# D-Hank/NeRF-tiny

Hardware: AMD Instinct MI355X
Metric: rays/sec (64 coarse + 128 fine samples), lego 400x400 (higher is better)
Workload: dtype f32

## Files before the change

### nerf-tiny_amd/csrc/field_fwd_reg.hip

```cpp
#include "field_common.h"
#include <type_traits>

namespace nerf {

constexpr int RM = 32;

template <int I0, int I1, class F>
__device__ __forceinline__ void static_for(F&& f) {
  if constexpr (I0 < I1) {
    f(std::integral_constant<int, I0>{});
    static_for<I0 + 1, I1>(f);
  }
}

template <int NFT>
struct WStage {
  float4 w[NFT];
};

template <int KB, int NFT>
__device__ __forceinline__ void stage_load(const float4* __restrict__ seg_lane, int kb, WStage<NFT>& s) {
#pragma unroll
  for (int f = 0; f < NFT; ++f) s.w[f] = seg_lane[(size_t)(f * KB + kb) * 64];
}

__device__ __forceinline__ float relu1(float x) { return __int_as_float(max(__float_as_int(x), 0)); }

__device__ __forceinline__ float f4c(const float4& v, int c) { return c == 0 ? v.x : (c == 1 ? v.y : (c == 2 ? v.z : v.w)); }

typedef int lds_i32 __attribute__((address_space(3), may_alias));
typedef int i32x4v __attribute__((ext_vector_type(4), may_alias));
typedef __attribute__((address_space(3))) i32x4v lds_i32x4;
constexpr int RELU_LDS_DWORDS = 2 * 4 * 64 * 4;
constexpr int COL_LDS_DWORDS = 3 * HALF + 4;
struct ReluLds {
  lds_i32* w;
  lds_i32* m[4];
};
__device__ __forceinline__ ReluLds relu_lds(lds_i32* base, int lane) {
  ReluLds L;
  L.w = base + 4 * lane;
#pragma unroll
  for (int c = 0; c < 4; ++c) L.m[c] = base + 4 * lane + ((c + (lane >> 3)) & 3);
  return L;
}
__device__ __forceinline__ float4 lds_ld4(const lds_i32* p) {
  const i32x4v v = *reinterpret_cast<const lds_i32x4*>(p);
  return make_float4(__int_as_float(v[0]), __int_as_float(v[1]), __int_as_float(v[2]), __int_as_float(v[3]));
}
template <typename DST>
__device__ __forceinline__ void relu_lds_op(const ReluLds& L, const f32x16& src, DST& dst, int dst0, int slot, int i) {
  const int g = i / 6, j = i - 6 * g, off = (slot * 4 + g) * 256;
  if (j == 0) {
    const i32x4v v = {__float_as_int(src[4 * g]), __float_as_int(src[4 * g + 1]), __float_as_int(src[4 * g + 2]), __float_as_int(src[4 * g + 3])};
    *reinterpret_cast<lds_i32x4*>(L.w + off) = v;
  } else if (j < 5) {
    __hip_atomic_fetch_max(L.m[j - 1] + off, 0, __ATOMIC_RELAXED, __HIP_MEMORY_SCOPE_WORKGROUP);
  } else {
    const i32x4v v = *reinterpret_cast<lds_i32x4*>(L.w + off);
#pragma unroll
    for (int c = 0; c < 4; ++c) dst[dst0 + c] = __int_as_float(v[c]);
  }
}

struct SaveIn {
  float* rows;
  uint16_t* mask;
};

__device__ __forceinline__ void bias_group(const float* b4h, int t, int g, f32x16& acc) {
  const float4 q = *reinterpret_cast<const float4*>(b4h + 32 * t + 8 * g);
  acc[4 * g + 0] = q.x;
  acc[4 * g + 1] = q.y;
  acc[4 * g + 2] = q.z;
  acc[4 * g + 3] = q.w;
}

template <int KB, int NFT, int NKB, int NNFT, bool ZERO_INIT, bool RELU_IN, int SAVE = 0, bool LDS_RELU = false, bool NEXT_RELU = false, int NEXT_BIAS = 0>
__device__ __forceinline__ void reg_layer(const int seg, const int next_seg , int lane,
                                          const f32x16* prev, f32x16* acc, WStage<8>& st0, const float* bv,
                                          const SaveIn sv, const RegBuf& rb, const ReluLds& rl, f32x4v& head,
                                          const float* nb = nullptr, f32x16* nacc = nullptr) {
  static_assert(!(LDS_RELU || NEXT_RELU || NEXT_BIAS) || SAVE != 1, "the saving forward keeps the VALU ReLU and the bias MFMAs");
  static_assert(NEXT_BIAS == 0 || ((LDS_RELU && RELU_IN) || NEXT_RELU), "the bias loads live in the stream with compile-time k-blocks");
  static_assert(NEXT_BIAS != 1 || (KB == 32 && RELU_IN), "NEXT_BIAS = 1 overwrites the 8 input tiles of a 256-wide ReLU layer");
  static_assert(NEXT_BIAS != 2 || KB == 8, "NEXT_BIAS = 2: one tile per k-block of layer 0");
  constexpr int KT = KB / 4;
  constexpr bool LR = LDS_RELU && RELU_IN;
  WStage<8> st1;
  const f32x16 zero = {0.f, 0.f, 0.f, 0.f, 0.f, 0.f, 0.f, 0.f, 0.f, 0.f, 0.f, 0.f, 0.f, 0.f, 0.f, 0.f};
  if (bv != nullptr) {
    const float one_h0 = (lane < 32) ? 1.0f : 0.0f;
#pragma unroll
    for (int f = 0; f < NFT; ++f) acc[f] = __builtin_amdgcn_mfma_f32_32x32x2f32(bv[f], one_h0, zero, 0, 0, 0);
  }
  f32x16 tin[2];
  if constexpr (LR) {
#pragma unroll
    for (int c = 0; c < 4; ++c) tin[0][c] = head[c];
    if (bv != nullptr) {
#pragma unroll
      for (int i = 6; i < 14; ++i) relu_lds_op(rl, prev[0], tin[0], 4 * (i / 6), 0, i);
#pragma unroll
      for (int i = 6; i < 14; ++i) {
        __builtin_amdgcn_sched_group_barrier(0x008, 1, 0);
        __builtin_amdgcn_sched_group_barrier(0x080, 1, 0);
      }
    }
  }
  [[maybe_unused]] const int lr0 = (bv != nullptr) ? 14 : 6;
  auto mask_word = [&](int t) {
    unsigned bits = 0;
#pragma unroll
    for (int r = 0; r < 16; ++r) bits |= (prev[t][r] > 0.f) ? (1u << r) : 0u;
    sv.mask[((t & 1) * 2) * 256 + (t >> 1) * 64] = (uint16_t)bits;
  };
  auto activate = [&](int t) {
    if constexpr (LR) {
      if (SAVE != 0) mask_word(t);
      return;
    }
#pragma unroll
    for (int r = 0; r < 16; ++r) tin[t & 1][r] = RELU_IN ? (SAVE == 1 ? fmaxf(prev[t][r], 0.f) : relu1(prev[t][r])) : prev[t][r];
#pragma unroll
    for (int r = 0; r < 16; ++r) asm volatile("" : "+v"(tin[t & 1][r]));
    if (SAVE == 1 || (SAVE == 2 && !RELU_IN)) {
#pragma unroll
      for (int g = 0; g < 4; ++g)
        store_row4(sv.rows + 32 * t + 8 * g, make_float4(tin[t & 1][4 * g], tin[t & 1][4 * g + 1], tin[t & 1][4 * g + 2], tin[t & 1][4 * g + 3]));
    }
    if (SAVE != 0 && RELU_IN) {
      unsigned bits = 0;
#pragma unroll
      for (int r = 0; r < 16; ++r) bits |= (prev[t][r] > 0.f) ? (1u << r) : 0u;
      sv.mask[((t & 1) * 2) * 256 + (t >> 1) * 64] = (uint16_t)bits;
    }
  };
  activate(0);
  if constexpr (!(LR || NEXT_RELU)) {
#pragma unroll
  for (int kb = 0; kb < KB; ++kb) {
    WStage<8>& ld = (kb & 1) ? st0 : st1;
    const WStage<8>& cur = (kb & 1) ? st1 : st0;
    if (kb + 1 < KB) {
#pragma unroll
      for (int f = 0; f < NFT; ++f) ld.w[f] = reg_ldw(rb, seg + (f * KB + kb + 1) * 64);
    } else if (next_seg >= 0) {
#pragma unroll
      for (int f = 0; f < NNFT; ++f) ld.w[f] = reg_ldw(rb, next_seg + (f * NKB) * 64);
    }
    __builtin_amdgcn_sched_barrier(0);
    if ((kb & 3) == 2 && (kb >> 2) + 1 < KT) activate((kb >> 2) + 1);
#pragma unroll
    for (int s = 0; s < 4; ++s) {
      const float b = tin[(kb >> 2) & 1][4 * (kb & 3) + s];
#pragma unroll
      for (int f = 0; f < NFT; ++f) {
        if (ZERO_INIT && bv == nullptr && kb == 0 && s == 0)
          acc[f] = __builtin_amdgcn_mfma_f32_32x32x2f32(f4c(cur.w[f], s), b, zero, 0, 0, 0);
        else
          acc[f] = __builtin_amdgcn_mfma_f32_32x32x2f32(f4c(cur.w[f], s), b, acc[f], 0, 0, 0);
      }
    }
  }
  } else {
  auto ds0 = [&](int kt, int k4, int s, int f) { const int i = lr0 + (k4 * 4 + s) * NFT + f; return (LR && kt == 0 && i < 24) ? i : -1; };
  auto ds1 = [&](int kt, int k4, int s, int f) { const int i = (k4 * 4 + s) * NFT + f - (NFT == 8 ? 64 : 16); return (LR && kt + 1 < KT && i >= 0 && i < 24) ? i : -1; };
  auto ds2 = [&](int kt, int k4, int s, int f) { return (NEXT_RELU && kt == KT - 1 && k4 == 3 && s == 3 && f < 6) ? f : -1; };
  auto nbt = [&](int kb, int s, int f) {
    if (NEXT_BIAS == 0 || s != 0 || f >= 4) return -1;
    if (NEXT_BIAS == 2) return kb;
    return kb == 1 ? 0 : (((kb & 3) == 3 && (kb >> 2) + 1 < KT) ? (kb >> 2) + 1 : -1);
  };
  static_for<0, KB>([&](auto kbc) __attribute__((always_inline)) {
    constexpr int kb = decltype(kbc)::value, kt = kb >> 2, k4 = kb & 3;
    WStage<8>& ld = (kb & 1) ? st0 : st1;
    const WStage<8>& cur = (kb & 1) ? st1 : st0;
    if (kb + 1 < KB) {
#pragma unroll
      for (int f = 0; f < NFT; ++f) ld.w[f] = reg_ldw(rb, seg + (f * KB + kb + 1) * 64);
    } else if (next_seg >= 0) {
#pragma unroll
      for (int f = 0; f < NNFT; ++f) ld.w[f] = reg_ldw(rb, next_seg + (f * NKB) * 64);
    }
    __builtin_amdgcn_sched_barrier(0);
    if (k4 == 2 && kt + 1 < KT) activate(kt + 1);
    bool any = false;
#pragma unroll
    for (int s = 0; s < 4; ++s) {
      const float b = tin[kt & 1][4 * k4 + s];
#pragma unroll
      for (int f = 0; f < NFT; ++f) {
        if (ZERO_INIT && bv == nullptr && kb == 0 && s == 0)
          acc[f] = __builtin_amdgcn_mfma_f32_32x32x2f32(f4c(cur.w[f], s), b, zero, 0, 0, 0);
        else
          acc[f] = __builtin_amdgcn_mfma_f32_32x32x2f32(f4c(cur.w[f], s), b, acc[f], 0, 0, 0);
        const int i0 = ds0(kt, k4, s, f), i1 = ds1(kt, k4, s, f), i2 = ds2(kt, k4, s, f);
        if constexpr (LR) {
          if (i0 >= 0) relu_lds_op(rl, prev[0], tin[0], 4 * (i0 / 6), 0, i0);
          if (i1 >= 0) relu_lds_op(rl, prev[kt + 1], tin[(kt + 1) & 1], 4 * (i1 / 6), (kt + 1) & 1, i1);
        }
        if constexpr (NEXT_RELU) {
          if (i2 >= 0) relu_lds_op(rl, acc[0], head, 0, 0, i2);
        }
        if constexpr (NEXT_BIAS != 0) {
          const int tb = nbt(kb, s, f);
          if (tb >= 0) bias_group(nb, tb, f, nacc[tb]);
          any |= tb >= 0;
        }
        any |= i0 >= 0 || i1 >= 0 || i2 >= 0;
      }
    }
    if (any) {
#pragma unroll
      for (int s = 0; s < 4; ++s)
#pragma unroll
        for (int f = 0; f < NFT; ++f) {
          const int n = (ds0(kt, k4, s, f) >= 0) + (ds1(kt, k4, s, f) >= 0) + (ds2(kt, k4, s, f) >= 0);
          __builtin_amdgcn_sched_group_barrier(0x008, 1, 0);
          if (n == 1) __builtin_amdgcn_sched_group_barrier(0x080, 1, 0);
          if (n == 2) __builtin_amdgcn_sched_group_barrier(0x080, 2, 0);
          if (nbt(kb, s, f) >= 0) __builtin_amdgcn_sched_group_barrier(0x020, 1, 0);
        }
    }
  });
  }
  if (KB & 1) st0 = st1;
}

template <int NFT>
__device__ __forceinline__ void bias_load(const float* __restrict__ bias, int lane, float (&bv)[8]) {
#pragma unroll
  for (int f = 0; f < NFT; ++f) bv[f] = bias[f * 32 + (lane & 31)];
}

#ifdef NERF_STAMPS
#define RSTAMP(slot)                                            \
  do {                                                          \
    __builtin_amdgcn_sched_barrier(0);                          \
    const unsigned long long t_ = __builtin_readcyclecounter(); \
    __builtin_amdgcn_sched_barrier(0);                          \
    tsum[slot] += t_ - tlast;                                   \
    tlast = t_;                                                 \
  } while (0)
#else
#define RSTAMP(slot) do { } while (0)
#endif

enum { SRC_RAYS = 0, SRC_POINTS = 1, SRC_LATTICE = 2, SRC_CORNERS = 3, SRC_BLOCKS = 4 };

template <bool SAVE, bool DEBUG, int SRC = SRC_RAYS, bool RGB = true, bool GSAVE = false>
__global__ __launch_bounds__(64, 1) void k_field_fwd_reg(const FieldArgs a, const QuerySrc q) {
#ifdef NERF_STAMPS
  unsigned long long tsum[12] = {0, 0, 0, 0, 0, 0, 0, 0, 0, 0, 0, 0};
  unsigned long long tlast = __builtin_readcyclecounter();
#endif
  const int lane = threadIdx.x, j = lane & 31, h = lane >> 5;
  const int m0 = blockIdx.x * RM;
  const int m = m0 + j;
  const bool valid = m < a.M;
  const int mc = valid ? m : a.M - 1;
  const int ray = (SRC == SRC_RAYS) ? mc / a.N : mc;
  const float* rf = (SRC == SRC_RAYS) ? a.rayf + (size_t)ray * RAYF : nullptr;
  const float4* wp = a.wp;
  const RegBuf rb = reg_buf(a.wp, threadIdx.x);

  WStage<8> st0;
  stage_load<8, 8>(wp + seg_off4(SEG_L0) + lane, 0, st0);
  constexpr bool LR = !SAVE;
  constexpr bool COL_LDS = LR && RGB;
  [[maybe_unused]] float4 cw0, cw1;
  [[maybe_unused]] float cb;
  if constexpr (COL_LDS) {
    const float4* wc4 = reinterpret_cast<const float4*>(a.w.p[W_COLOR]);
    cw0 = wc4[lane];
    cw1 = wc4[64 + j];
    cb = a.w.p[B_COLOR][lane < 3 ? lane : 2];
  }

  float p[3];
  [[maybe_unused]] bool band_keep = false;
  [[maybe_unused]] size_t band_at = 0;
  if constexpr (SRC == SRC_RAYS) {
    sample_point(rf, a.t[mc], p);
  } else if constexpr (SRC == SRC_POINTS) {
#pragma unroll
    for (int c = 0; c < 3; ++c) p[c] = q.points[(size_t)mc * 3 + c];
  } else if constexpr (SRC == SRC_LATTICE) {
    const int iz = mc % q.nz, ixy = mc / q.nz;
    const int iy = ixy % q.ny, ix = ixy / q.ny;
    p[0] = q.lo[0] + (float)ix * q.step[0];
    p[1] = q.lo[1] + (float)iy * q.step[1];
    p[2] = q.lo[2] + (float)iz * q.step[2];
  } else {
    static_assert(!RGB && !SAVE && !GSAVE && !DEBUG, "the band forms are sigma-only inference");
    const unsigned n[3] = {(unsigned)q.nx, (unsigned)q.ny, (unsigned)q.nz};
    unsigned idx[3];
    band_keep = valid;
    if constexpr (SRC == SRC_CORNERS) {
      const unsigned uz = (unsigned)mc % (unsigned)q.ext[2], uxy = (unsigned)mc / (unsigned)q.ext[2];
      idx[0] = uxy / (unsigned)q.ext[1] * (unsigned)q.r;
      idx[1] = uxy % (unsigned)q.ext[1] * (unsigned)q.r;
      idx[2] = uz * (unsigned)q.r;
    } else {
      const unsigned vol = (unsigned)(q.ext[0] * q.ext[1] * q.ext[2]);
      const unsigned e = (unsigned)mc / vol, l = (unsigned)mc - e * vol;
      band_keep = band_keep && (long long)q.e0 + e < *q.nlist;
      const unsigned b = band_keep ? (unsigned)q.list[(size_t)q.e0 + e] : 0u;
      const unsigned lz = l % (unsigned)q.ext[2], lxy = l / (unsigned)q.ext[2];
      const unsigned bz = b % (unsigned)q.nbz, bxy = b / (unsigned)q.nbz;
      idx[0] = bxy / (unsigned)q.nby * (unsigned)q.r + lxy / (unsigned)q.ext[1];
      idx[1] = bxy % (unsigned)q.nby * (unsigned)q.r + lxy % (unsigned)q.ext[1];
      idx[2] = bz * (unsigned)q.r + lz;
      band_keep = band_keep && idx[0] < n[0] && idx[1] < n[1] && idx[2] < n[2];
    }
#pragma unroll
    for (int c = 0; c < 3; ++c) idx[c] = idx[c] < n[c] ? idx[c] : n[c] - 1u;
    band_at = ((size_t)idx[0] * n[1] + idx[1]) * n[2] + idx[2];
    p[0] = q.lo[0] + (float)(int)idx[0] * q.step[0];
    p[1] = q.lo[1] + (float)(int)idx[1] * q.step[1];
    p[2] = q.lo[2] + (float)(int)idx[2] * q.step[2];
  }
  if (DEBUG && a.pts_dbg && valid && h == 0) {
    a.pts_dbg[(size_t)m * 3 + 0] = p[0];
    a.pts_dbg[(size_t)m * 3 + 1] = p[1];
    a.pts_dbg[(size_t)m * 3 + 2] = p[2];
  }
  f32x16 gp[2];
  static_for<0, 16>([&](auto ic) __attribute__((always_inline)) {
    constexpr int g8 = decltype(ic)::value >> 1, e = decltype(ic)::value & 1;
    constexpr int pa = 4 * g8 + e, pb = pa + 2;
    constexpr bool pad = pb >= 30;
    constexpr int ca = pa / 10, la = pa - 10 * ca, cb = pad ? ca : pb / 10, lb = pad ? la : pb - 10 * cb;
    static_assert(pa < 30, "lane half 0 never pads");
    constexpr uint32_t fa = kFreqPointLit[la], fb = kFreqPointLit[lb];
    const float x = (ca == cb) ? p[ca] : (h ? p[cb] : p[ca]);
    const float f = (la == lb) ? __uint_as_float(fa) : (h ? __uint_as_float(fb) : __uint_as_float(fa));
    float sv, cv;
    sincos_phase(x * f, sv, cv);
    if (pad) {
      sv = h ? 0.f : sv;
      cv = h ? 0.f : cv;
    }
    gp[g8 >> 2][4 * (g8 & 3) + 2 * e] = sv;
    gp[g8 >> 2][4 * (g8 & 3) + 2 * e + 1] = cv;
  });
  if (DEBUG && a.gp_dbg && valid) {
#pragma unroll
    for (int g8 = 0; g8 < 8; ++g8)
#pragma unroll
      for (int s = 0; s < 4; ++s) {
        const int k = 8 * g8 + 4 * h + s;
        if (k < POINT_DIM) a.gp_dbg[(size_t)m * POINT_DIM + k] = gp[g8 >> 2][4 * (g8 & 3) + s];
      }
  }

  const size_t MS = (size_t)a.MSrows * WIDTH;
  const long long rrow = valid ? (long long)(a.row0 + m) : a.Mtot + j;
  float* const srow = SAVE ? a.save + (size_t)rrow * WIDTH + 4 * h : nullptr;
  uint16_t* const mrow = (SAVE || GSAVE) ? a.masks + ((size_t)(a.tile0 + (m0 >> 6)) * 4 + ((m0 >> 5) & 1)) * 256 + h * 32 + j : nullptr;
  const size_t MKS = (size_t)a.tiles_tot * 4 * 256;
  auto sv_rows = [&](int tensor) { return SaveIn{SAVE ? srow + (size_t)tensor * MS : nullptr, nullptr}; };
  auto sv_relu = [&](int layer) { return SaveIn{SAVE ? srow + (size_t)layer * MS : nullptr, SAVE ? mrow + (size_t)layer * MKS : nullptr}; };
  float* const gprow = GSAVE ? a.save + (size_t)rrow * QGRAD_GP + 4 * h : nullptr;
  float* const crow = GSAVE ? a.save + (size_t)a.MSrows * QGRAD_GP + (size_t)rrow * QGRAD_C + 4 * h : nullptr;
  constexpr int SV = SAVE ? 1 : (GSAVE ? 2 : 0);
  auto sv_in = [&](int layer) { return GSAVE ? SaveIn{nullptr, mrow + (size_t)layer * MKS} : sv_relu(layer); };

  ReluLds rl{};
  [[maybe_unused]] lds_i32* col = nullptr;
  if constexpr (LR) {
    __shared__ int relu_slots[RELU_LDS_DWORDS + (COL_LDS ? COL_LDS_DWORDS : 0)];
    rl = relu_lds((lds_i32*)relu_slots, lane);
    if constexpr (COL_LDS) {
      col = (lds_i32*)relu_slots + RELU_LDS_DWORDS;
      const i32x4v v0 = {__float_as_int(cw0.x), __float_as_int(cw0.y), __float_as_int(cw0.z), __float_as_int(cw0.w)};
      const i32x4v v1 = {__float_as_int(cw1.x), __float_as_int(cw1.y), __float_as_int(cw1.z), __float_as_int(cw1.w)};
      *reinterpret_cast<lds_i32x4*>(col + 4 * lane) = v0;
      *reinterpret_cast<lds_i32x4*>(col + 4 * (64 + j)) = v1;
      col[3 * HALF + (lane < 3 ? lane : 2)] = __float_as_int(cb);
    }
  }
  f32x4v head = {0.f, 0.f, 0.f, 0.f};
  RSTAMP(0);
  f32x16 A[8], B[8];
  constexpr int L256 = 8 * 32 * 64;
  constexpr int sL1 = seg_off4(SEG_L1);
  constexpr int sL5 = seg_off4(SEG_L5);
  float bv[8];
  constexpr bool BL = LR;
  constexpr int NB1 = BL ? 1 : 0;
  auto bl = [&](int i) { return BL ? a.w.p[i] + 4 * h : nullptr; };
  auto bias_mfma = [&](int i) -> const float* {
    if constexpr (BL) return nullptr;
    bias_load<8>(a.w.p[i], lane, bv);
    return bv;
  };
  if constexpr (BL) {
#pragma unroll
    for (int t = 0; t < 8; ++t)
#pragma unroll
      for (int g = 0; g < 4; ++g) bias_group(bl(B_L0), t, g, A[t]);
  }

  reg_layer<8, 8, 32, 8, !BL, false, SV, LR, LR, BL ? 2 : 0>(seg_off4(SEG_L0), sL1, lane, gp, A, st0, bias_mfma(B_L0), GSAVE ? SaveIn{gprow, nullptr} : sv_rows(S_GP), rb, rl, head, bl(3), B);
  RSTAMP(1);
  reg_layer<32, 8, 32, 8, !BL, true, SV, LR, LR, NB1>(sL1, sL1 + L256, lane, A, B, st0, bias_mfma(3), sv_in(0), rb, rl, head, bl(5), A);
  reg_layer<32, 8, 32, 8, !BL, true, SV, LR, LR, NB1>(sL1 + L256, sL1 + 2 * L256, lane, B, A, st0, bias_mfma(5), sv_in(1), rb, rl, head, bl(7), B);
  reg_layer<32, 8, 32, 8, !BL, true, SV, LR, LR, NB1>(sL1 + 2 * L256, seg_off4(SEG_L4A), lane, A, B, st0, bias_mfma(7), sv_in(2), rb, rl, head, bl(9), A);
  RSTAMP(2);
  reg_layer<32, 8, 8, 8, !BL, true, SV, LR, false, NB1>(seg_off4(SEG_L4A), seg_off4(SEG_L4B), lane, B, A, st0, bias_mfma(9), sv_in(3), rb, rl, head, bl(11), B);
  reg_layer<8, 8, 32, 8, false, false, 0, LR, LR>(seg_off4(SEG_L4B), sL5, lane, gp, A, st0, nullptr, SaveIn{nullptr, nullptr}, rb, rl, head);
  RSTAMP(3);
  reg_layer<32, 8, 32, 8, !BL, true, SV, LR, LR, NB1>(sL5, sL5 + L256, lane, A, B, st0, bias_mfma(11), sv_in(4), rb, rl, head, bl(13), A);
  reg_layer<32, 8, 32, 8, !BL, true, SV, LR, LR, NB1>(sL5 + L256, sL5 + 2 * L256, lane, B, A, st0, bias_mfma(13), sv_in(5), rb, rl, head, bl(15), B);
  reg_layer<32, 8, 32, 4, !BL, true, SV, LR, false>(sL5 + 2 * L256, RGB ? seg_off4(SEG_FOLD) : -1, lane, A, B, st0, bias_mfma(15), sv_in(6), rb, rl, head);
  RSTAMP(4);
  {
    const float* ws = a.w.p[W_SIGMA] + 4 * h;
    float s = 0.f;
    float4 wq[2][4];
#pragma unroll
    for (int g = 0; g < 4; ++g) wq[0][g] = *reinterpret_cast<const float4*>(ws + 8 * g);
#pragma unroll
    for (int t = 0; t < 8; ++t) {
      if (t + 1 < 8) {
#pragma unroll
        for (int g = 0; g < 4; ++g) wq[(t + 1) & 1][g] = *reinterpret_cast<const float4*>(ws + 32 * (t + 1) + 8 * g);
      }
      if (SAVE) __builtin_amdgcn_sched_barrier(0);
      if (GSAVE) {
        unsigned bits = 0;
#pragma unroll
        for (int r = 0; r < 16; ++r) bits |= (B[t][r] > 0.f) ? (1u << r) : 0u;
        mrow[7 * MKS + ((t & 1) * 2) * 256 + (t >> 1) * 64] = (uint16_t)bits;
      }
#pragma unroll
      for (int g = 0; g < 4; ++g) {
        const float4 q = wq[t & 1][g];
        s = __builtin_fmaf(relu1(B[t][4 * g + 0]), q.x, s);
        s = __builtin_fmaf(relu1(B[t][4 * g + 1]), q.y, s);
        s = __builtin_fmaf(relu1(B[t][4 * g + 2]), q.z, s);
        s = __builtin_fmaf(relu1(B[t][4 * g + 3]), q.w, s);
      }
      if (SAVE) __builtin_amdgcn_sched_barrier(0);
    }
    s += __shfl_xor(s, 32);
    if constexpr (SRC == SRC_CORNERS || SRC == SRC_BLOCKS) {
      if (band_keep && h == 0) a.sigma[band_at] = fabsf(s + a.w.p[B_SIGMA][0]);
    } else if (valid && h == 0) {
      const float pre = s + a.w.p[B_SIGMA][0];
      a.sigma[m] = fabsf(pre);
      if (SAVE || GSAVE) a.spre[a.row0 + m] = pre;
    }
  }
  RSTAMP(5);
  if constexpr (!RGB) return;
  {
    const float* dv = a.dvec + (size_t)ray * HALF + 4 * h;
#pragma unroll
    for (int f = 0; f < 4; ++f)
#pragma unroll
      for (int g = 0; g < 4; ++g) {
        const float4 q = *reinterpret_cast<const float4*>(dv + 32 * f + 8 * g);
        A[f][4 * g + 0] = q.x;
        A[f][4 * g + 1] = q.y;
        A[f][4 * g + 2] = q.z;
        A[f][4 * g + 3] = q.w;
      }
  }
  reg_layer<32, 4, 32, 4, false, true, SAVE, false, false>(seg_off4(SEG_FOLD), -1, lane, B, A, st0, nullptr, GSAVE ? SaveIn{nullptr, nullptr} : sv_relu(7), rb, rl, head);
  RSTAMP(6);
  {
    const float* wc = a.w.p[W_COLOR] + 4 * h;
    float z0 = 0.f, z1 = 0.f, z2 = 0.f;
#pragma unroll
    for (int t = 0; t < 4; ++t)
#pragma unroll
      for (int g = 0; g < 4; ++g) {
        float4 q0, q1, q2;
        if constexpr (COL_LDS) {
          q0 = lds_ld4(col + 4 * h + 32 * t + 8 * g);
          q1 = lds_ld4(col + 4 * h + HALF + 32 * t + 8 * g);
          q2 = lds_ld4(col + 4 * h + 2 * HALF + 32 * t + 8 * g);
        } else {
          q0 = *reinterpret_cast<const float4*>(wc + 32 * t + 8 * g);
          q1 = *reinterpret_cast<const float4*>(wc + HALF + 32 * t + 8 * g);
          q2 = *reinterpret_cast<const float4*>(wc + 2 * HALF + 32 * t + 8 * g);
        }
        const float c0 = relu1(A[t][4 * g + 0]), c1 = relu1(A[t][4 * g + 1]);
        const float c2 = relu1(A[t][4 * g + 2]), c3 = relu1(A[t][4 * g + 3]);
        if (SAVE) store_row4(srow + S_C * MS + 32 * t + 8 * g, make_float4(c0, c1, c2, c3));
        if (GSAVE) store_row4(crow + 32 * t + 8 * g, make_float4(c0, c1, c2, c3));
        z0 = __builtin_fmaf(c3, q0.w, __builtin_fmaf(c2, q0.z, __builtin_fmaf(c1, q0.y, __builtin_fmaf(c0, q0.x, z0))));
        z1 = __builtin_fmaf(c3, q1.w, __builtin_fmaf(c2, q1.z, __builtin_fmaf(c1, q1.y, __builtin_fmaf(c0, q1.x, z1))));
        z2 = __builtin_fmaf(c3, q2.w, __builtin_fmaf(c2, q2.z, __builtin_fmaf(c1, q2.y, __builtin_fmaf(c0, q2.x, z2))));
      }
    z0 += __shfl_xor(z0, 32);
    z1 += __shfl_xor(z1, 32);
    z2 += __shfl_xor(z2, 32);
    float bc[3];
    if constexpr (COL_LDS) {
      const float4 b = lds_ld4(col + 3 * HALF);
      bc[0] = b.x, bc[1] = b.y, bc[2] = b.z;
    }
    if (valid && h == 0) {
      if constexpr (!COL_LDS) {
#pragma unroll
        for (int c = 0; c < 3; ++c) bc[c] = a.w.p[B_COLOR][c];
      }
      a.rgb[(size_t)m * 3 + 0] = 1.0f / (1.0f + expf(-(z0 + bc[0])));
      a.rgb[(size_t)m * 3 + 1] = 1.0f / (1.0f + expf(-(z1 + bc[1])));
      a.rgb[(size_t)m * 3 + 2] = 1.0f / (1.0f + expf(-(z2 + bc[2])));
    }
  }
#ifdef NERF_STAMPS
  RSTAMP(7);
  if (a.stamps && lane == 0) {
    for (int i = 0; i < 8; ++i) atomicAdd(a.stamps + i, tsum[i]);
    atomicAdd(a.stamps + 31, 1ull);
  }
#endif
}

hipError_t launch_field_fwd_reg(const FieldArgs& a, bool save, hipStream_t st) {
  const int tiles = (a.M + RM - 1) / RM;
  if (save)
    hipLaunchKernelGGL((k_field_fwd_reg<true, false>), dim3(tiles), dim3(64), 0, st, a, QuerySrc{});
  else if (a.pts_dbg || a.gp_dbg)
    hipLaunchKernelGGL((k_field_fwd_reg<false, true>), dim3(tiles), dim3(64), 0, st, a, QuerySrc{});
  else
    hipLaunchKernelGGL((k_field_fwd_reg<false, false>), dim3(tiles), dim3(64), 0, st, a, QuerySrc{});
  return hipGetLastError();
}

hipError_t launch_query_grad_fwd(const FieldArgs& a, const QuerySrc& q, bool rgb, hipStream_t st) {
  if (a.M <= 0) return hipSuccess;
  const unsigned tiles = (unsigned)(((long long)a.M + RM - 1) / RM);
  if (rgb)
    hipLaunchKernelGGL((k_field_fwd_reg<false, false, SRC_POINTS, true, true>), dim3(tiles), dim3(64), 0, st, a, q);
  else
    hipLaunchKernelGGL((k_field_fwd_reg<false, false, SRC_POINTS, false, true>), dim3(tiles), dim3(64), 0, st, a, q);
  return hipGetLastError();
}

hipError_t launch_query_reg(const FieldArgs& a, const QuerySrc& q, bool rgb, hipStream_t st) {
  if (a.M <= 0) return hipSuccess;
  const unsigned tiles = (unsigned)(((long long)a.M + RM - 1) / RM);
  if (q.points == nullptr)
    hipLaunchKernelGGL((k_field_fwd_reg<false, false, SRC_LATTICE, false>), dim3(tiles), dim3(64), 0, st, a, q);
  else if (rgb)
    hipLaunchKernelGGL((k_field_fwd_reg<false, false, SRC_POINTS, true>), dim3(tiles), dim3(64), 0, st, a, q);
  else
    hipLaunchKernelGGL((k_field_fwd_reg<false, false, SRC_POINTS, false>), dim3(tiles), dim3(64), 0, st, a, q);
  return hipGetLastError();
}

hipError_t launch_band_corners(const FieldArgs& a, const QuerySrc& q, hipStream_t st) {
  if (a.M <= 0) return hipSuccess;
  hipLaunchKernelGGL((k_field_fwd_reg<false, false, SRC_CORNERS, false>), dim3((unsigned)(((long long)a.M + RM - 1) / RM)), dim3(64), 0, st, a, q);
  return hipGetLastError();
}

hipError_t launch_band_blocks(const FieldArgs& a, const QuerySrc& q, hipStream_t st) {
  if (a.M <= 0) return hipSuccess;
  hipLaunchKernelGGL((k_field_fwd_reg<false, false, SRC_BLOCKS, false>), dim3((unsigned)(((long long)a.M + RM - 1) / RM)), dim3(64), 0, st, a, q);
  return hipGetLastError();
}

}
```

Baseline: 737,700.

## Fuse sigma head into fold layer using LDS ReLU round trip and LDS weights

In the non-saving RGB forward, the sigma output head is no longer a separate pass after layer 7. The fold layer now runs in LDS-ReLU mode and accumulates the sigma dot product from the ReLU'd input tiles that the LDS round trip brings back, with the sigma weights staged in LDS and the bias packed into the colour-bias slot. The aim is to drop the standalone sigma loop with its global weight loads and hide that work under the MFMA stream. The cost is extra LDS space, extra VALU FMAs and DS loads inside the scheduled MFMA loop, and a change in which layer does its ReLU through LDS.

```diff
diff --git a/nerf-tiny_amd/csrc/field_fwd_reg.hip b/nerf-tiny_amd/csrc/field_fwd_reg.hip
--- a/nerf-tiny_amd/csrc/field_fwd_reg.hip
+++ b/nerf-tiny_amd/csrc/field_fwd_reg.hip
@@ -33,6 +33,12 @@
 typedef __attribute__((address_space(3))) i32x4v lds_i32x4;
 constexpr int RELU_LDS_DWORDS = 2 * 4 * 64 * 4;
 constexpr int COL_LDS_DWORDS = 3 * HALF + 4;
+constexpr int SIG_LDS_DWORDS = WIDTH;
+struct SigmaTap {
+  const lds_i32* ws;
+  float4 wq[4];
+  float s;
+};
 struct ReluLds {
   lds_i32* w;
   lds_i32* m[4];
@@ -76,12 +82,13 @@
   acc[4 * g + 3] = q.w;
 }
 
-template <int KB, int NFT, int NKB, int NNFT, bool ZERO_INIT, bool RELU_IN, int SAVE = 0, bool LDS_RELU = false, bool NEXT_RELU = false, int NEXT_BIAS = 0>
+template <int KB, int NFT, int NKB, int NNFT, bool ZERO_INIT, bool RELU_IN, int SAVE = 0, bool LDS_RELU = false, bool NEXT_RELU = false, int NEXT_BIAS = 0, bool TAP = false>
 __device__ __forceinline__ void reg_layer(const int seg, const int next_seg , int lane,
                                           const f32x16* prev, f32x16* acc, WStage<8>& st0, const float* bv,
                                           const SaveIn sv, const RegBuf& rb, const ReluLds& rl, f32x4v& head,
-                                          const float* nb = nullptr, f32x16* nacc = nullptr) {
+                                          const float* nb = nullptr, f32x16* nacc = nullptr, SigmaTap* tap = nullptr) {
   static_assert(!(LDS_RELU || NEXT_RELU || NEXT_BIAS) || SAVE != 1, "the saving forward keeps the VALU ReLU and the bias MFMAs");
+  static_assert(!TAP || (LDS_RELU && RELU_IN && NFT == 4), "the tap reads the tiles that the LDS round trip brings back; its DS slots are those of NFT = 4");
   static_assert(NEXT_BIAS == 0 || ((LDS_RELU && RELU_IN) || NEXT_RELU), "the bias loads live in the stream with compile-time k-blocks");
   static_assert(NEXT_BIAS != 1 || (KB == 32 && RELU_IN), "NEXT_BIAS = 1 overwrites the 8 input tiles of a 256-wide ReLU layer");
   static_assert(NEXT_BIAS != 2 || KB == 8, "NEXT_BIAS = 2: one tile per k-block of layer 0");
@@ -167,6 +174,7 @@
   auto ds0 = [&](int kt, int k4, int s, int f) { const int i = lr0 + (k4 * 4 + s) * NFT + f; return (LR && kt == 0 && i < 24) ? i : -1; };
   auto ds1 = [&](int kt, int k4, int s, int f) { const int i = (k4 * 4 + s) * NFT + f - (NFT == 8 ? 64 : 16); return (LR && kt + 1 < KT && i >= 0 && i < 24) ? i : -1; };
   auto ds2 = [&](int kt, int k4, int s, int f) { return (NEXT_RELU && kt == KT - 1 && k4 == 3 && s == 3 && f < 6) ? f : -1; };
+  auto ds3 = [&](int k4, int s, int f) { return (TAP && k4 == 2 && s == 2) ? f : -1; };
   auto nbt = [&](int kb, int s, int f) {
     if (NEXT_BIAS == 0 || s != 0 || f >= 4) return -1;
     if (NEXT_BIAS == 2) return kb;
@@ -185,6 +193,12 @@
     }
     __builtin_amdgcn_sched_barrier(0);
     if (k4 == 2 && kt + 1 < KT) activate(kt + 1);
+    if constexpr (TAP && k4 == 3) {
+#pragma unroll
+      for (int g = 0; g < 4; ++g)
+#pragma unroll
+        for (int r = 0; r < 4; ++r) tap->s = __builtin_fmaf(tin[kt & 1][4 * g + r], f4c(tap->wq[g], r), tap->s);
+    }
     bool any = false;
 #pragma unroll
     for (int s = 0; s < 4; ++s) {
@@ -203,12 +217,16 @@
         if constexpr (NEXT_RELU) {
           if (i2 >= 0) relu_lds_op(rl, acc[0], head, 0, 0, i2);
         }
+        const int i3 = ds3(k4, s, f);
+        if constexpr (TAP) {
+          if (i3 >= 0) tap->wq[i3] = lds_ld4(tap->ws + 32 * kt + 8 * i3);
+        }
         if constexpr (NEXT_BIAS != 0) {
           const int tb = nbt(kb, s, f);
           if (tb >= 0) bias_group(nb, tb, f, nacc[tb]);
           any |= tb >= 0;
         }
-        any |= i0 >= 0 || i1 >= 0 || i2 >= 0;
+        any |= i0 >= 0 || i1 >= 0 || i2 >= 0 || i3 >= 0;
       }
     }
     if (any) {
@@ -216,7 +234,7 @@
       for (int s = 0; s < 4; ++s)
 #pragma unroll
         for (int f = 0; f < NFT; ++f) {
-          const int n = (ds0(kt, k4, s, f) >= 0) + (ds1(kt, k4, s, f) >= 0) + (ds2(kt, k4, s, f) >= 0);
+          const int n = (ds0(kt, k4, s, f) >= 0) + (ds1(kt, k4, s, f) >= 0) + (ds2(kt, k4, s, f) >= 0) + (ds3(k4, s, f) >= 0);
           __builtin_amdgcn_sched_group_barrier(0x008, 1, 0);
           if (n == 1) __builtin_amdgcn_sched_group_barrier(0x080, 1, 0);
           if (n == 2) __builtin_amdgcn_sched_group_barrier(0x080, 2, 0);
@@ -269,13 +287,15 @@
   stage_load<8, 8>(wp + seg_off4(SEG_L0) + lane, 0, st0);
   constexpr bool LR = !SAVE;
   constexpr bool COL_LDS = LR && RGB;
-  [[maybe_unused]] float4 cw0, cw1;
+  constexpr bool H7_LDS = COL_LDS && !GSAVE;
+  [[maybe_unused]] float4 cw0, cw1, sw;
   [[maybe_unused]] float cb;
   if constexpr (COL_LDS) {
     const float4* wc4 = reinterpret_cast<const float4*>(a.w.p[W_COLOR]);
     cw0 = wc4[lane];
     cw1 = wc4[64 + j];
-    cb = a.w.p[B_COLOR][lane < 3 ? lane : 2];
+    cb = (H7_LDS && lane == 3) ? a.w.p[B_SIGMA][0] : a.w.p[B_COLOR][lane < 3 ? lane : 2];
+    if constexpr (H7_LDS) sw = reinterpret_cast<const float4*>(a.w.p[W_SIGMA])[lane];
   }
 
   float p[3];
@@ -369,8 +389,9 @@
 
   ReluLds rl{};
   [[maybe_unused]] lds_i32* col = nullptr;
+  [[maybe_unused]] lds_i32* sig = nullptr;
   if constexpr (LR) {
-    __shared__ int relu_slots[RELU_LDS_DWORDS + (COL_LDS ? COL_LDS_DWORDS : 0)];
+    __shared__ int relu_slots[RELU_LDS_DWORDS + (COL_LDS ? COL_LDS_DWORDS : 0) + (H7_LDS ? SIG_LDS_DWORDS : 0)];
     rl = relu_lds((lds_i32*)relu_slots, lane);
     if constexpr (COL_LDS) {
       col = (lds_i32*)relu_slots + RELU_LDS_DWORDS;
@@ -378,7 +399,12 @@
       const i32x4v v1 = {__float_as_int(cw1.x), __float_as_int(cw1.y), __float_as_int(cw1.z), __float_as_int(cw1.w)};
       *reinterpret_cast<lds_i32x4*>(col + 4 * lane) = v0;
       *reinterpret_cast<lds_i32x4*>(col + 4 * (64 + j)) = v1;
-      col[3 * HALF + (lane < 3 ? lane : 2)] = __float_as_int(cb);
+      col[3 * HALF + ((lane < 3 || (H7_LDS && lane == 3)) ? lane : 2)] = __float_as_int(cb);
+      if constexpr (H7_LDS) {
+        sig = col + COL_LDS_DWORDS;
+        const i32x4v v2 = {__float_as_int(sw.x), __float_as_int(sw.y), __float_as_int(sw.z), __float_as_int(sw.w)};
+        *reinterpret_cast<lds_i32x4*>(sig + 4 * lane) = v2;
+      }
     }
   }
   f32x4v head = {0.f, 0.f, 0.f, 0.f};
@@ -414,9 +440,9 @@
   RSTAMP(3);
   reg_layer<32, 8, 32, 8, !BL, true, SV, LR, LR, NB1>(sL5, sL5 + L256, lane, A, B, st0, bias_mfma(11), sv_in(4), rb, rl, head, bl(13), A);
   reg_layer<32, 8, 32, 8, !BL, true, SV, LR, LR, NB1>(sL5 + L256, sL5 + 2 * L256, lane, B, A, st0, bias_mfma(13), sv_in(5), rb, rl, head, bl(15), B);
-  reg_layer<32, 8, 32, 4, !BL, true, SV, LR, false>(sL5 + 2 * L256, RGB ? seg_off4(SEG_FOLD) : -1, lane, A, B, st0, bias_mfma(15), sv_in(6), rb, rl, head);
+  reg_layer<32, 8, 32, 4, !BL, true, SV, LR, H7_LDS>(sL5 + 2 * L256, RGB ? seg_off4(SEG_FOLD) : -1, lane, A, B, st0, bias_mfma(15), sv_in(6), rb, rl, head);
   RSTAMP(4);
-  {
+  if constexpr (!H7_LDS) {
     const float* ws = a.w.p[W_SIGMA] + 4 * h;
     float s = 0.f;
     float4 wq[2][4];
@@ -469,7 +495,16 @@
         A[f][4 * g + 3] = q.w;
       }
   }
-  reg_layer<32, 4, 32, 4, false, true, SAVE, false, false>(seg_off4(SEG_FOLD), -1, lane, B, A, st0, nullptr, GSAVE ? SaveIn{nullptr, nullptr} : sv_relu(7), rb, rl, head);
+  [[maybe_unused]] float sig_s = 0.f;
+  if constexpr (H7_LDS) {
+    SigmaTap tap;
+    tap.ws = sig + 4 * h;
+    tap.s = 0.f;
+    reg_layer<32, 4, 32, 4, false, true, 0, true, false, 0, true>(seg_off4(SEG_FOLD), -1, lane, B, A, st0, nullptr, SaveIn{nullptr, nullptr}, rb, rl, head, nullptr, nullptr, &tap);
+    sig_s = tap.s + __shfl_xor(tap.s, 32);
+  } else {
+    reg_layer<32, 4, 32, 4, false, true, SAVE, false, false>(seg_off4(SEG_FOLD), -1, lane, B, A, st0, nullptr, GSAVE ? SaveIn{nullptr, nullptr} : sv_relu(7), rb, rl, head);
+  }
   RSTAMP(6);
   {
     const float* wc = a.w.p[W_COLOR] + 4 * h;
@@ -503,8 +538,10 @@
     if constexpr (COL_LDS) {
       const float4 b = lds_ld4(col + 3 * HALF);
       bc[0] = b.x, bc[1] = b.y, bc[2] = b.z;
+      if constexpr (H7_LDS) sig_s += b.w;
     }
     if (valid && h == 0) {
+      if constexpr (H7_LDS) a.sigma[m] = fabsf(sig_s);
       if constexpr (!COL_LDS) {
 #pragma unroll
         for (int c = 0; c < 3; ++c) bc[c] = a.w.p[B_COLOR][c];
```

Result: no change. 738,300, median of 5 (+0.1%).
